# multiplefish/VPLines-SLAM

Measured on AMD Instinct MI355X. Metric: sliding-window BA solves/sec (10 KF, 200 pts + 80 lines, 5 iters), higher is better.
Workload: dtype f64

## Files before the change

vplines-slam_amd/csrc/ba_ctx.h:

```cpp
#pragma once
#include <functional>
#include <map>
#include <string>

#include "vplines_ba.h"
#include "ba_types.h"
#include "ba_stage.h"

struct vpl_ctx {
  int device = 0;
  hipStream_t stream = nullptr;
  DevBatch B;
  std::vector<DevAlloc> allocs;
  bool guards = false;
  std::string err;
  int maxW = 0, maxP = 0, maxPO = 0, maxL = 0, maxLO = 0;
  int nW = 0;
  vpl_ba_options opt;
  bool upload_open = false;
  std::vector<int> h_nP, h_nL;
  std::vector<std::vector<int>> h_lmap;
  std::vector<int> h_mg_m;
  std::vector<int> h_mg_n;
  std::vector<int> h_mg_nb;
  std::vector<int> h_passthrough;
  std::vector<vpl_prior> h_pass_priors;
  bool any_second_new = false;
  int maxPriorN = 0;
  bool prior_resident = false;
  int prior_resident_nW = 0;
  std::vector<int> layout_key;
  bool layout_valid = false;
  bool force_general = false;
  bool schur_mostly_wide = false;
  bool schur_never_wide = false;
  bool schur_wide_all = false;
  bool step_fused = true;
  size_t marg_smem = 0;
  int marg_nmax = 0;
  bool marg_small = false;
  int prior_rule = VPL_PRIOR_PIVOTED_CHOLESKY;
  hipGraphExec_t graph_exec = nullptr;
  bool use_graph = true;
  bool timing = false;
  std::map<std::string, std::pair<double, int>> ktimes;
  std::vector<std::pair<const char*, double>> ltimes;
  int* d_act = nullptr;
  std::vector<std::string> kname_store;
  bool leg_timing = false;
  hipEvent_t leg_ev[6] = {nullptr, nullptr, nullptr, nullptr, nullptr, nullptr};
  double odo_ms[3] = {0, 0, 0};
  std::function<int()> pending;
  Stage stage;
  size_t last_upload_bytes = 0;
  struct vpl_odo* odo = nullptr;
};

static void drop_graph(vpl_ctx* c) {
  if (c->graph_exec) { (void)hipGraphExecDestroy(c->graph_exec); c->graph_exec = nullptr; }
}

static int settle(vpl_ctx* c) {
  if (!c || !c->pending) return VPL_OK;
  std::function<int()> fin;
  fin.swap(c->pending);
  return fin();
}
static int finish_or_defer(vpl_ctx* c, bool async, std::function<int()> fin) {
  if (!async) return fin();
  c->pending = std::move(fin);
  return VPL_OK;
}

struct KTimer {
  vpl_ctx* c;
  const char* name;
  hipEvent_t a = nullptr, b = nullptr;
  KTimer(vpl_ctx* c_, const char* n) : c(c_), name(n) {
    if (c->timing) { (void)hipEventCreate(&a); (void)hipEventCreate(&b); (void)hipEventRecord(a, c->stream); }
  }
  ~KTimer() {
    if (c->timing) {
      (void)hipEventRecord(b, c->stream);
      (void)hipEventSynchronize(b);
      float ms = 0;
      (void)hipEventElapsedTime(&ms, a, b);
      auto& e = c->ktimes[name];
      e.first += ms;
      e.second += 1;
// ... 14 lines not shown
```

vplines-slam_amd/csrc/ba_lin.h:

```cpp
#pragma once
#include "ba_common.h"

namespace vpl {

typedef double v4d_lin __attribute__((ext_vector_type(4)));
constexpr int LIN_THREADS = 512;
constexpr int STG_LD = 17;
constexpr int LIN_STAGE = 8 * 32 * STG_LD;
constexpr int PRE_LDS = 62;
constexpr int LIN_HW = 720;
constexpr int PREP_NMAX = 112;
__host__ __device__ constexpr int lin_stage_doubles(int maxL) {
  const int ln = 8 * LIN_HW + 38 * maxL;
  const int pt = LIN_STAGE + 78 * 36 + NV;
  const int m = ln > pt ? ln : pt;
  return m > 4650 + 3570 ? m : 4650 + 3570;
}
constexpr int PREP_THREADS = 640;
inline size_t prep_smem(int max_prior_n) {
  const int ns = max_prior_n < PREP_NMAX ? max_prior_n : PREP_NMAX;
  return (size_t)((PREP_THREADS / 64) * 675 + ns * ns) * sizeof(double);
}
constexpr size_t PREP_SMEM = (size_t)((PREP_THREADS / 64) * 675 + PREP_NMAX * PREP_NMAX) * sizeof(double);

__device__ __forceinline__ void prep_body(const DevBatch& B, const int w, double* psm, int nstage) {
  const int tid = threadIdx.x;
  const int lane = tid & 63, wv = tid >> 6;
  const int NWV = blockDim.x >> 6;
  double* wsc = psm + wv * 675;
  double* Jl = psm + NWV * 675;
  const int n = B.pr_n[w];
  const bool fits = n > 0 && n <= nstage;
  if (fits) {
    const double* J0g = B.pr_J0 + (size_t)w * B.prS;
    for (int idx = tid; idx < n * n; idx += blockDim.x) Jl[idx] = J0g[idx];
  }
  for (int j = 1 + wv; j < NF; j += NWV) {
    DevPreint& P = B.pre[(size_t)w * NF + j];
    double* G = wsc;
    double* X = wsc + 225;
    double* Pm = wsc + 450;
    for (int k = lane; k < 225; k += 64) G[k] = P.cov[k];
    __builtin_amdgcn_wave_barrier();
    wave_chol16(G, 15, 15, X, lane);
    __builtin_amdgcn_wave_barrier();
    for (int e = lane; e < 225; e += 64) {
      const int a = e / 15, b2 = e % 15;
      double s2 = 0;
      for (int k = (a > b2 ? a : b2); k < 15; ++k) s2 += X[k * 15 + a] * X[k * 15 + b2];
      Pm[e] = s2;
    }
    __builtin_amdgcn_wave_barrier();
    wave_chol16(Pm, 15, 15, nullptr, lane);
    __builtin_amdgcn_wave_barrier();
    for (int e = lane; e < 225; e += 64) {
      const int i = e / 15, jj = e % 15;
      P.sqrt_info[e] = (jj >= i) ? Pm[jj * 15 + i] : 0.0;
    }
    __builtin_amdgcn_wave_barrier();
  }
  if (tid < NF + 1) {
    double* x = tid < NF ? B.pose + ((size_t)w * NF + tid) * 7 : B.ex + (size_t)w * 7;
    Q4 q = mat2q(qmat(qnormalized(qpose(x))));
    if (tid == 0) {
      M3 R0 = qmat(qnormalized(qpose(x)));
      V3 ypr = R2ypr(R0);
      double* g = B.gauge + (size_t)w * 4;
      g[0] = ypr.x; g[1] = x[0]; g[2] = x[1]; g[3] = x[2];
      const double* fr = B.fail_ref + (size_t)w * 13;
      if (fr[0] != 0.0) {
        M3 Rl;
        for (int k = 0; k < 9; ++k) Rl.m[k] = fr[4 + k];
        g[0] = R2ypr(Rl).x; g[1] = fr[1]; g[2] = fr[2]; g[3] = fr[3];
      }
    }
    x[3] = q.x; x[4] = q.y; x[5] = q.z; x[6] = q.w;
    double* xq = psm + 7 * tid;
    xq[0] = x[0]; xq[1] = x[1]; xq[2] = x[2]; xq[3] = q.x; xq[4] = q.y; xq[5] = q.z; xq[6] = q.w;
  }
  __syncthreads();
  const int nL = B.orth_in[w] ? 0 : B.nL[w];
  for (int l = tid; l < nL; l += blockDim.x) {
    const int s = B.ln_start[(size_t)w * B.maxL + l];
    const double* ps = psm + 7 * s;
    const double* ex = psm + 7 * NF;
    M3 Rs = qmat(qpose(ps)), ric = qmat(qpose(ex));
    V3 P{ps[0], ps[1], ps[2]}, tic{ex[0], ex[1], ex[2]};
    V3 twc = P + mul(Rs, tic);
    M3 Rwc = mul(Rs, ric);
    const double* pl = B.plk + ((size_t)w * B.maxL + l) * 6;
    Plk Lc{V3{pl[0], pl[1], pl[2]}, V3{pl[3], pl[4], pl[5]}};
    Plk Lw = plk_to_pose(Lc, Rwc, twc);
    plk_to_orth(Lw, B.orth + ((size_t)w * B.maxL + l) * 4);
  }
  for (int l = tid; l < B.nL[w]; l += blockDim.x) {
    const size_t li = (size_t)w * B.maxL + l;
    const Plk Lw = orth_to_plk(B.orth + li * 4);
    double* o = B.lw + li * 6;
    o[0] = Lw.n.x; o[1] = Lw.n.y; o[2] = Lw.n.z; o[3] = Lw.v.x; o[4] = Lw.v.y; o[5] = Lw.v.z;
  }
  if (n > 0) {
    const double* J0 = B.pr_J0 + (size_t)w * B.prS;
    double* H = B.pr_H + (size_t)w * B.prS;
    const double* Js = fits ? Jl : J0;
    if (fits) {
      const int NT = (n + 15) >> 4, NLT = NT * (NT + 1) / 2, KS = (n + 3) >> 2;
      const int m = lane & 15, kk = lane >> 4;
      for (int t = wv; t < NLT; t += NWV) {
        int ta, tb;
        tri_decode(t, ta, tb);
        const int ca = 16 * ta + m, cb = 16 * tb + m;
        v4d_lin acc = {0, 0, 0, 0};
        for (int ks = 0; ks < KS; ++ks) {
          const int k = 4 * ks + kk;
          const double av = (k < n && ca < n) ? Js[k * n + ca] : 0.0;
          const double bv = (k < n && cb < n) ? Js[k * n + cb] : 0.0;
          acc = __builtin_amdgcn_mfma_f64_16x16x4f64(av, bv, acc, 0, 0, 0);
        }
        const double vals[4] = {acc.x, acc.y, acc.z, acc.w};
#pragma unroll
        for (int v = 0; v < 4; ++v) {
          const int r = 16 * ta + kk + 4 * v, c2 = cb;
          if (r < n && c2 < n && (ta != tb || r >= c2)) {
            H[(size_t)r * n + c2] = vals[v];
            H[(size_t)c2 * n + r] = vals[v];
          }
        }
      }
    } else
    for (int idx = tid; idx < n * n; idx += blockDim.x) {
      int a = idx / n, b = idx % n;
      double s = 0;
      for (int k = 0; k < n; ++k) s += Js[(size_t)k * n + a] * Js[(size_t)k * n + b];
      H[idx] = s;
    }
    for (int c2 = tid; c2 < n; c2 += blockDim.x) {
      double s = 0;
      const double* r0g = B.pr_r0 + (size_t)w * MAXPN;
#pragma unroll 8
      for (int k = 0; k < n; ++k) s += Js[(size_t)k * n + c2] * r0g[k];
      B.pr_g0[(size_t)w * MAXPN + c2] = s;
    }
    if (tid < B.pr_nb[w]) {
      int kind = B.pr_kind[(size_t)w * MAXPB + tid], fr = B.pr_frame[(size_t)w * MAXPB + tid];
      int idx = B.pr_idx[(size_t)w * MAXPB + tid];
      int base = kind == 0 ? 15 * fr : kind == 1 ? 15 * fr + 6 : 165;
      int ls = kind == 1 ? 9 : 6;
      for (int k = 0; k < ls; ++k) B.pr_map[(size_t)w * MAXPN + idx + k] = base + k;
    }
  }
  if (tid == 0) {
    TrState t;
    t.radius = 1e4; t.mu = 1e-8; t.x_cost = 0; t.cand_cost = 0; t.model_cost_change = 0; t.x_norm = 0;
    t.step_norm = 0; t.dogleg_step_norm = 0; t.alpha = 0; t.a1 = t.a2 = t.a3 = 0; t.initial_cost = 0;
    t.iter = 0; t.status = 0; t.reuse = 0; t.step_valid = 0; t.fresh_lin = 0; t.num_successful = 0; t.num_invalid = 0;
    t.pad = 0;
    B.tr[w] = t;
  }
}
__global__ __launch_bounds__(PREP_THREADS) void k_prep(DevBatch B, int nstage) {
  extern __shared__ double psm[];
  prep_body(B, blockIdx.x, psm, nstage);
}

constexpr int HV_DOUBLES = 78 * 36;
constexpr int LIN_PART = 78 * 36 + 72 + 8;
__host__ __device__ __forceinline__ int hvi(int r, int c) {
  const int br = r / 6, bc = c / 6;
  return 36 * (br * (br + 1) / 2 + bc) + 6 * (r - 6 * br) + (c - 6 * bc);
}

inline void lin_asm_entry(int r, int c, int* out) {
  int hv = 0, im = 0;
  const int vr = cam2vis(r), vc = cam2vis(c);
  if (vr >= 0 && vc >= 0) hv = hvi(vr, vc) + 1;
  if (r < 165) {
    const int fr = r / 15, ar = r - 15 * fr, fc = c / 15, bc = c - 15 * fc;
    if (fc == fr) im = 120 * fr + ar * (ar + 1) / 2 + bc + 1;
    else if (fc == fr - 1) im = 11 * 120 + 225 * (fr - 1) + 15 * ar + bc + 1;
  }
  out[0] = hv | im << 16;
  out[1] = r | c << 8;
}

template <int MODE, int ROLE>
// ... 775 lines not shown
```

vplines-slam_amd/csrc/ba_upload.h:

```cpp
#pragma once
#include "ba_ctx.h"
#include "ba_odo.h"
#include "ba_pack.h"
#include "host_common.h"

static void to_dev_preint(const vpl_preintegration& p, DevPreint& d) {
  d.sum_dt = p.sum_dt;
  for (int k = 0; k < 3; ++k) { d.dp[k] = p.delta_p[k]; d.dv[k] = p.delta_v[k]; d.lba[k] = p.linearized_ba[k]; d.lbg[k] = p.linearized_bg[k]; }
  for (int k = 0; k < 4; ++k) d.dq[k] = p.delta_q[k];
  auto blk = [&](double* o, int r0, int c0) {
    for (int i = 0; i < 3; ++i)
      for (int j = 0; j < 3; ++j) o[3 * i + j] = p.jacobian[(r0 + i) * 15 + c0 + j];
  };
  blk(d.dp_dba, 0, 9); blk(d.dp_dbg, 0, 12); blk(d.dq_dbg, 3, 12); blk(d.dv_dba, 6, 9); blk(d.dv_dbg, 6, 12);
  std::memcpy(d.cov, p.covariance, sizeof(d.cov));
  std::memset(d.sqrt_info, 0, sizeof(d.sqrt_info));
}

struct UploadArena {
  Span<double> pose, sb, ex, invd, plk, pt_obs, ln_obs, fail_ref, orth, pr_x0, pr_r0;
  Span<int> nP, nL, pt_start, pt_nobs, pt_off, ln_start, ln_nobs, ln_off, ln_tri, pu_cnt, pu_cnt0, sk_tab, sk_wave, path, nLO, lo_ln,
      ll_tab, ll_np, ps_list, ps_cnt, orth_in, pr_n, pr_nb, pr_kind, pr_frame, pr_idx, mg_n, mg_nb, mg_kind, mg_frame, mg_idx, mg_cam, mg_m;
  Span<DevPreint> pre;
  std::vector<Span<double>> J0;
// ... 86 lines not shown
    for (size_t w = 0; w < W; ++w) S.put(B.pr_J0 + w * (size_t)B.prS, A.J0[w]);
  }
  S.put(B.mg_n, A.mg_n); S.put(B.mg_nb, A.mg_nb); S.put(B.mg_kind, A.mg_kind);
  S.put(B.mg_frame, A.mg_frame); S.put(B.mg_idx, A.mg_idx); S.put(B.mg_cam, A.mg_cam); S.put(B.mg_m, A.mg_m);
  S.put(B.path, A.path);
}
static size_t upload_bound(const DevBatch& B, size_t W, const vpl_window* win, bool same_layout, bool chained, const OdoSrc* odo) {
  Stage dry;
  dry.dry = true;
  UploadArena A;
  take_upload(dry, A, B, W, win, chained, odo);
  take_units(dry, A, W, B.maxPR);
  stage_upload(dry, A, B, W, same_layout, chained, odo);
  return dry.bound();
}

static int upload_check(vpl_ctx* c, int nW, const vpl_window* win, const vpl_ba_options* opt, bool chained) {
  if (!c || !win || !opt || nW < 1) return VPL_E_INVALID;
  if (nW > c->maxW) return fail(c, VPL_E_CAPACITY, "more windows than max_windows");
  if (opt->marginalization_flag != VPL_MARGIN_OLD && opt->marginalization_flag != VPL_MARGIN_SECOND_NEW &&
      opt->marginalization_flag != VPL_MARGIN_NONE)
    return fail(c, VPL_E_INVALID, "unknown marginalization_flag");
  HIPCHK(c, hipSetDevice(c->device));
  { const int rs = settle(c); if (rs) return rs; }
  if (chained && (!c->prior_resident || c->prior_resident_nW != nW))
    return fail(c, VPL_E_INVALID, "upload_chained: needs a previous solve of the same batch size with a marginalisation, and no upload since");
  return VPL_OK;
}

static int read_resident_priors(vpl_ctx* c, size_t W, std::vector<HostTab>& tab) {
  const DevBatch& B = c->B;
  int* const src[10] = {B.mg_n, B.mg_nb, B.mg_kind, B.mg_frame, B.mg_idx, B.pr_n, B.pr_nb, B.pr_kind, B.pr_frame, B.pr_idx};
  Span<int> t[10];
  auto plan = [&](Stage& S) {
    for (int k = 0; k < 10; ++k) {
      t[k] = S.take<int>(k % 5 < 2 ? W : W * MAXPB);
      S.from_device(t[k].p, src[k], t[k].n);
    }
  };
  HIPCHK(c, stage_plan(c->stage, plan));
  HIPCHK(c, stage_run(c->stage, c->stream, false));
  HIPCHK(c, hipStreamSynchronize(c->stream));
  tab.resize(W);
  for (size_t w = 0; w < W; ++w) {
    HostTab& T = tab[w];
    T.keep = c->h_passthrough[w] >= 0;
    const Span<int>* s = t + (T.keep ? 5 : 0);
// ... 258 lines not shown
  DevBuf dkeep;
  HIPCHK(c, dkeep.alloc(nW * 4));
  HIPCHK(c, hipMemcpyAsync(dkeep.p, keep.data(), nW * 4, hipMemcpyHostToDevice, c->stream));
  if (B.prS != prev_prS && std::any_of(keep.begin(), keep.end(), [](int k) { return k != 0; })) {
    DevBuf tmp;
    HIPCHK(c, tmp.alloc(nW * (size_t)MAXPN * MAXPN * 8));
    hipLaunchKernelGGL(k_prior_restride, dim3(nW), dim3(256), 0, c->stream, B, (const int*)dkeep.p, prev_prS, tmp.d(), 0);
    hipLaunchKernelGGL(k_prior_restride, dim3(nW), dim3(256), 0, c->stream, B, (const int*)dkeep.p, prev_prS, tmp.d(), 1);
    HIPCHK(c, hipGetLastError());
    HIPCHK(c, hipStreamSynchronize(c->stream));
  }
  hipLaunchKernelGGL(k_prior_handoff, dim3(nW), dim3(256), 0, c->stream, B, (const int*)dkeep.p);
  HIPCHK(c, hipGetLastError());
  HIPCHK(c, hipStreamSynchronize(c->stream));
  return VPL_OK;
}

static int upload_body(vpl_ctx* c, int nW, const vpl_window* win, const vpl_ba_options* opt, bool all_lines, bool chained,
                       const OdoSrc* odo) {
  int rc = upload_check(c, nW, win, opt, chained);
  if (rc) return rc;
  const int prev_prS = c->B.prS;
  c->prior_resident = false;
  if (c->leg_timing) HIPCHK(c, hipEventRecord(c->leg_ev[0], c->stream));
  drop_graph(c);
  c->upload_open = true;
  c->opt = *opt;
  c->nW = nW;
  DevBatch& B = c->B;
  B.nW = nW;
  B.opt.num_iterations = opt->num_iterations;
  B.opt.estimate_extrinsic = opt->estimate_extrinsic;
  B.opt.marginalization_flag = opt->marginalization_flag;
  B.opt.remove_line_outliers = opt->remove_line_outliers;
  B.opt.sqrt_info_point = opt->focal_length / 1.5;
  B.opt.sqrt_info_line = opt->line_factor;
  B.opt.sqrt_info_vp = opt->vp_factor;
  B.opt.g_norm = opt->g_norm;
  B.opt.huber_delta = opt->huber_delta;
  const size_t W = nW;
  std::vector<HostTab> ctab;
  if (chained && (rc = read_resident_priors(c, W, ctab))) return rc;
  const bool dev_prior = chained || odo;
  if (odo) {
    ctab.assign(W, HostTab());
    for (size_t w = 0; w < W; ++w)
// ... 39 lines not shown
  if (SG.overflow) return fail(c, VPL_E_CAPACITY, "internal: staging arena bound too small");
  stage_upload(SG, A, B, W, same_layout, dev_prior, odo);
  if (chained && (rc = hand_over_priors(c, ctab, prev_prS))) return rc;
  HIPCHK(c, stage_run(c->stage, c->stream, true, &c->last_upload_bytes));
  if (odo) {
    hipLaunchKernelGGL(k_odo_gather, dim3(nW), dim3(ODO_THREADS), 0, c->stream, B, odo->store, (const int*)odo->d_psrc, (const int*)odo->d_lsrc);
    if (odo->tab) hipLaunchKernelGGL(k_odo_prior_load, dim3(nW), dim3(ODO_THREADS), 0, c->stream, B, odo->prior, (const int*)odo->d_has);
    HIPCHK(c, hipGetLastError());
  }
  if (c->leg_timing) HIPCHK(c, hipEventRecord(c->leg_ev[1], c->stream));
  HIPCHK(c, hipStreamSynchronize(c->stream));
  c->layout_valid = true;
  return VPL_OK;
}
static int upload_impl(vpl_ctx* c, int nW, const vpl_window* win, const vpl_ba_options* opt, bool all_lines, bool chained = false,
                       const OdoSrc* odo = nullptr) {
  const int rc = upload_body(c, nW, win, opt, all_lines, chained, odo);
  if (c) {
    if (rc != VPL_OK && c->upload_open) { c->nW = 0; c->prior_resident = false; }
    c->upload_open = false;
  }
  return rc;
}

static int restore_states(vpl_ctx* c, bool plk) {
  const DevBatch& B = c->B;
  const size_t W = c->nW;
  HIPCHK(c, hipMemcpyAsync(B.pose, B.pose_0, W * 77 * 8, hipMemcpyDeviceToDevice, c->stream));
  HIPCHK(c, hipMemcpyAsync(B.sb, B.sb_0, W * 99 * 8, hipMemcpyDeviceToDevice, c->stream));
  HIPCHK(c, hipMemcpyAsync(B.ex, B.ex_0, W * 7 * 8, hipMemcpyDeviceToDevice, c->stream));
  HIPCHK(c, hipMemcpyAsync(B.invd, B.invd_0, W * B.maxP * 8, hipMemcpyDeviceToDevice, c->stream));
  if (plk) HIPCHK(c, hipMemcpyAsync(B.plk, B.plk_0, W * B.maxL * 6 * 8, hipMemcpyDeviceToDevice, c->stream));
  return VPL_OK;
}
```

vplines-slam_amd/csrc/vplines_ba.hip:

```cpp
#include <hip/hip_runtime.h>

#include <algorithm>
#include <chrono>
#include <memory>
#include <cstdlib>
#include <cstring>
#include <string>
#include <vector>

#include "vplines_ba.h"
#include "ba_types.h"
#include "ba_lin.h"
#include "ba_pack.h"
#include "ba_solve.h"
#include "ba_step.h"
#include "ba_marg.h"
#include "ba_prior_eig.h"
#include "ba_lineopt.h"
#include "ba_factors.h"
#include "ba_odo.h"
#include "odo_tracks.h"
#include "host_common.h"

using namespace vpl;
// ... 138 lines not shown
      }
    if ((int)nz.size() != NZ_N || hipMemcpy(B.nz_tab, nz.data(), nz.size() * sizeof(int), hipMemcpyHostToDevice) != hipSuccess) return VPL_E_HIP;
  }
  static size_t lin_max = 0, solve_max = 0, schur_max = 0, back_max = 0, step_max = 0;
  lin_max = std::max(lin_max, lin_smem(c->maxP, c->maxL));
  solve_max = std::max(solve_max, solve_smem(c->maxP, c->maxL));
  schur_max = std::max(schur_max, schur_smem(c->maxP, c->maxL));
  back_max = std::max(back_max, back_smem(c->maxP, c->maxL));
  step_max = std::max(step_max, step_smem(c->maxP, c->maxL));
  if (schur_max > 159 * 1024 || back_max > 159 * 1024) return VPL_E_CAPACITY;
  const std::pair<const void*, size_t> lds[] = {
      {(const void*)k_lin2, lin_max}, {(const void*)k_lin<1>, lin_max}, {(const void*)k_lin<2>, lin_max},
      {(const void*)k_solve, solve_max}, {(const void*)k_schur<3>, schur_max}, {(const void*)k_schur<5>, schur_max},
      {(const void*)k_schur_mixed, schur_max}, {(const void*)k_chol, CHOL_SMEM}, {(const void*)k_back, back_max},
      {(const void*)k_step<3, false>, step_max}, {(const void*)k_step<3, true>, step_max}, {(const void*)k_step<5, false>, step_max},
      {(const void*)k_prep, PREP_SMEM}, {(const void*)k_marg<MARG_THREADS>, 159 * 1024}, {(const void*)k_marg<256>, MARG_LDS_SMALL},
      {(const void*)k_prior_eigen, prior_eig_layout(MAXKEEP).bytes}, {(const void*)k_init_align, init_lds_bytes(INIT_NMAX)}};
  for (const auto& k : lds)
    if (hipFuncSetAttribute(k.first, hipFuncAttributeMaxDynamicSharedMemorySize, (int)k.second) != hipSuccess) return VPL_E_HIP;
  vpl_ba_default_options(&c->opt);
  if (const char* gv = std::getenv("VPL_BA_GRAPH")) c->use_graph = std::atoi(gv) != 0;
  if (const char* gv = std::getenv("VPL_BA_GENERAL")) c->force_general = std::atoi(gv) != 0;
  if (const char* gv = std::getenv("VPL_BA_STEP_FUSED")) c->step_fused = std::atoi(gv) != 0;
  if (const char* gv = std::getenv("VPL_BA_SCHUR_WIDE")) { c->schur_wide_all = std::atoi(gv) > 0; c->schur_never_wide = std::atoi(gv) < 0; }
  return VPL_OK;
}

int vpl_ctx_create(vpl_ctx** out, int device, int max_windows, int max_points, int max_point_obs, int max_lines,
                   int max_line_obs) {
  if (!out || max_windows < 1 || max_points < 0 || max_lines < 0) return VPL_E_INVALID;
  int ndev = 0;
  if (hipGetDeviceCount(&ndev) != hipSuccess || ndev == 0 || device >= ndev) return VPL_E_NODEVICE;
  if (hipSetDevice(device) != hipSuccess) return VPL_E_NODEVICE;
  vpl_ctx* c = new vpl_ctx();
  const int rc = ctx_init(c, device, max_windows, max_points, max_point_obs, max_lines, max_line_obs);
  if (rc != VPL_OK) {
    free_arrays(c);
    delete c;
    return rc;
  }
  *out = c;
  return VPL_OK;
}

void vpl_ctx_destroy(vpl_ctx* c) {
  if (!c) return;
  (void)hipSetDevice(c->device);
  (void)hipDeviceSynchronize();
  drop_graph(c);
  free_arrays(c);
  c->stage.release();
  for (hipEvent_t& e : c->leg_ev) if (e) (void)hipEventDestroy(e);
  delete c;
}

int vpl_ctx_set_stream(vpl_ctx* c, void* s) {
  if (!c) return VPL_E_INVALID;
  const int rs = settle(c);
  if (rs) return rs;
  if (c->stream != (hipStream_t)s) {
    HIPCHK(c, hipSetDevice(c->device));
    (void)hipStreamSynchronize(c->stream);
    (void)hipGetLastError();
  }
  drop_graph(c);
  c->stream = (hipStream_t)s;
  return VPL_OK;
}
int vpl_ba_set_prior_rule(vpl_ctx* c, int rule) {
  if (!c || (rule != VPL_PRIOR_PIVOTED_CHOLESKY && rule != VPL_PRIOR_EIGEN)) return VPL_E_INVALID;
  const int rs = settle(c);
  if (rs) return rs;
  drop_graph(c);
  c->prior_rule = rule;
  return VPL_OK;
}
const char* vpl_last_error(const vpl_ctx* c) { return c ? c->err.c_str() : "null context"; }

int vpl_ctx_enable_leg_timing(vpl_ctx* c, int enable) {
  if (!c) return VPL_E_INVALID;
  HIPCHK(c, hipSetDevice(c->device));
  if (enable)
    for (hipEvent_t& e : c->leg_ev) if (!e) HIPCHK(c, hipEventCreate(&e));
  c->leg_timing = enable != 0;
  return VPL_OK;
}
int vpl_ctx_leg_times(vpl_ctx* c, double* ms3) {
  if (!c || !ms3 || !c->leg_timing) return VPL_E_INVALID;
  HIPCHK(c, hipSetDevice(c->device));
  HIPCHK(c, hipStreamSynchronize(c->stream));
// ... 107 lines not shown
  HIPCHK(c, hipMemcpyAsync(dJ.p, pr->J0, (size_t)n * n * 8, hipMemcpyHostToDevice, c->stream));
  HIPCHK(c, hipMemcpyAsync(dr0.p, pr->r0, n * 8, hipMemcpyHostToDevice, c->stream));
  HIPCHK(c, hipMemcpyAsync(dp.p, params, psz * 8, hipMemcpyHostToDevice, c->stream));
  hipLaunchKernelGGL(k_eval_prior, dim3(1), dim3(256), 0, c->stream, n, nb, (const int*)dk.p, (const int*)di.p, dx0.d(),
                     dJ.d(), dr0.d(), dp.d(), dr.d(), jac ? dj.d() : nullptr);
  HIPCHK(c, hipGetLastError());
  HIPCHK(c, hipMemcpyAsync(residuals, dr.p, n * 8, hipMemcpyDeviceToHost, c->stream));
  if (jac) HIPCHK(c, hipMemcpyAsync(jac, dj.p, (size_t)n * psz * 8, hipMemcpyDeviceToHost, c->stream));
  HIPCHK(c, hipStreamSynchronize(c->stream));
  return VPL_OK;
}
int vpl_pose_plus(vpl_ctx* c, int n, const double* x, const double* delta, double* out) {
  return eval_generic(c, n, x, 7, delta, 6, 7, 0, out, nullptr, [&](double* p, double* k, double* r, double*) {
    hipLaunchKernelGGL(k_eval_pose_plus, dim3((n + 63) / 64), dim3(64), 0, c->stream, n, p, k, r);
  });
}
int vpl_line_orth_plus(vpl_ctx* c, int n, const double* x, const double* delta, double* out) {
  return eval_generic(c, n, x, 4, delta, 4, 4, 0, out, nullptr, [&](double* p, double* k, double* r, double*) {
    hipLaunchKernelGGL(k_eval_orth_plus, dim3((n + 63) / 64), dim3(64), 0, c->stream, n, p, k, r);
  });
}

int vpl_ba_reset_state(vpl_ctx* c) {
  if (c) { const int rs = settle(c); if (rs) return rs; }
  if (!c || c->nW < 1) return VPL_E_INVALID;
  return restore_states(c, true);
}

int vpl_ba_upload(vpl_ctx* c, int nW, const vpl_window* win, const vpl_ba_options* opt) {
  return upload_impl(c, nW, win, opt, false);
}
int vpl_ba_upload_chained(vpl_ctx* c, int nW, const vpl_window* win, const vpl_ba_options* opt) {
  return upload_impl(c, nW, win, opt, false, true);
}

static void launch_prep(vpl_ctx* c, const DevBatch& B, int nw, hipStream_t s) {
  KTimer t(c, "k_prep");
  hipLaunchKernelGGL(k_prep, dim3(nw), dim3(PREP_THREADS), prep_smem(c->maxPriorN), s, B, std::min(c->maxPriorN, PREP_NMAX));
}
static void launch_marg(vpl_ctx* c, DevBatch& B, int nw, hipStream_t s) {
  const bool old = c->opt.marginalization_flag == VPL_MARGIN_OLD;
  if (!old && !c->any_second_new) return;
  const dim3 grid(nw);
  { KTimer t(c, "k_lin_marg");
    if (old) hipLaunchKernelGGL(k_lin<1>, grid, dim3(LIN_THREADS), lin_smem(c->maxP, c->maxL), s, B);
    else hipLaunchKernelGGL(k_lin<2>, grid, dim3(LIN_THREADS), lin_smem(c->maxP, c->maxL), s, B); }
  ++B.launch;
  { KTimer t(c, "k_marg");
    if (c->marg_small) hipLaunchKernelGGL(k_marg<256>, grid, dim3(256), c->marg_smem, s, B);
    else hipLaunchKernelGGL(k_marg<MARG_THREADS>, grid, dim3(MARG_THREADS), c->marg_smem, s, B); }
  if (c->prior_rule == VPL_PRIOR_EIGEN) {
    KTimer t(c, "k_prior_eigen");
    hipLaunchKernelGGL(k_prior_eigen, grid, dim3(PRIOR_EIG_THREADS), prior_eig_layout(c->marg_nmax).bytes, s, B, c->marg_nmax);
  }
}
static void launch_triangulate(vpl_ctx* c, int nW, bool points, bool lines, double init_depth) {
  const DevBatch& B = c->B;
  hipStream_t s = c->stream;
  if (points) { KTimer t(c, "k_triangulate_points"); hipLaunchKernelGGL(k_triangulate_points, dim3(nW), dim3(128), 0, s, B, init_depth); }
  if (lines) { KTimer t(c, "k_triangulate"); hipLaunchKernelGGL(k_triangulate, dim3(nW), dim3(128), 0, s, B); }
}
// ... 190 lines not shown
    for (size_t w = 0; w < W; ++w) {
      vpl_window& v = win[w];
      if (reports) std::memset(&reports[w], 0, sizeof(reports[w]));
      if (c->h_lmap[w].size() < 4) {
        if (v.line_removed) std::fill(v.line_removed, v.line_removed + v.n_lines, 0);
        continue;
      }
      const int nrem = scatter_solved_lines(c, w, v, &(*plk)[w * maxL * 6], &(*removed)[w * maxL]);
      if (reports) {
        fill_report(reports[w], (*tr)[w]);
        reports[w].n_lines_removed = nrem;
      }
    }
    return VPL_OK;
  });
}
int vpl_ba_only_line_opt(vpl_ctx* c, int nW, vpl_window* win, const vpl_ba_options* opt, vpl_solve_report* reports) {
  return only_line_opt_impl(c, nW, win, opt, reports, false);
}
int vpl_ba_only_line_opt_async(vpl_ctx* c, int nW, vpl_window* win, const vpl_ba_options* opt, vpl_solve_report* reports) {
  return only_line_opt_impl(c, nW, win, opt, reports, true);
}

static void launch_solve(vpl_ctx* c, int w0, int nw, hipStream_t s) {
  DevBatch B = c->B;
  B.ord_it = 0;
  B.act = c->timing ? c->d_act : nullptr;
  B.launch = 0;
  B.step_fused = c->step_fused && !c->timing;
  if (c->timing) { c->ltimes.clear(); (void)hipMemsetAsync(c->d_act, 0, sizeof(int) * ACT_SLOTS * 4, s); }
  const dim3 grid(nw);
  launch_prep(c, B, nw, s);
  ++B.launch;
  { KTimer t(c, "k_lin"); hipLaunchKernelGGL(k_lin2, dim3(16 * ((nw + 7) / 8)), dim3(LIN_THREADS), lin_smem(c->maxP, c->maxL), s, B); }
  ++B.launch;
  for (int it = 0; it < c->opt.num_iterations; ++it) {
    B.ord_it = it;
    const bool wide = c->schur_wide_all || (c->schur_mostly_wide && !c->schur_never_wide);
    if (B.step_fused) {
      if (B.WS + 2 <= 48) hipLaunchKernelGGL((k_step<3, false>), grid, dim3(SCHUR_THREADS), step_smem(B.maxP, B.maxL, 3), s, B);
      else if (wide) hipLaunchKernelGGL((k_step<5, false>), grid, dim3(SCHUR_THREADS), step_smem(B.maxP, B.maxL, 5), s, B);
      else hipLaunchKernelGGL((k_step<3, true>), grid, dim3(SCHUR_THREADS), step_smem(B.maxP, B.maxL, 3), s, B);
      ++B.launch;
      hipLaunchKernelGGL(k_solve, grid, dim3(SOLVE_THREADS), solve_smem(B.maxP, B.maxL), s, B);
      ++B.launch;
    } else {
      { KTimer t(c, "k_schur");
        if (B.WS + 2 <= 48) hipLaunchKernelGGL(k_schur<3>, grid, dim3(SCHUR_THREADS), schur_smem(B.maxP, B.maxL, 3), s, B);
        else if (wide) hipLaunchKernelGGL(k_schur<5>, grid, dim3(SCHUR_THREADS), schur_smem(B.maxP, B.maxL, 5), s, B);
        else hipLaunchKernelGGL(k_schur_mixed, grid, dim3(SCHUR_THREADS), schur_smem(B.maxP, B.maxL, 3), s, B); }
      ++B.launch;
      { KTimer t(c, "k_chol"); hipLaunchKernelGGL(k_chol, grid, dim3(CHOL_THREADS), CHOL_SMEM, s, B); }
      ++B.launch;
      { KTimer t(c, "k_solve"); hipLaunchKernelGGL(k_solve, grid, dim3(SOLVE_THREADS), solve_smem(B.maxP, B.maxL), s, B); }
      ++B.launch;
      { KTimer t(c, "k_back"); hipLaunchKernelGGL(k_back, grid, dim3(BACK_THREADS), back_smem(B.maxP, B.maxL), s, B); }
      ++B.launch;
    }
    { KTimer t(c, "k_cost"); hipLaunchKernelGGL(k_cost, grid, dim3(COST_THREADS), 0, s, B); }
    ++B.launch;
    if (it + 1 < c->opt.num_iterations) {
      B.ord_it = it + 1;
      KTimer t(c, "k_lin");
      hipLaunchKernelGGL(k_lin2, dim3(16 * ((nw + 7) / 8)), dim3(LIN_THREADS), lin_smem(c->maxP, c->maxL), s, B);
    }
    if (it + 1 < c->opt.num_iterations) ++B.launch;
  }
  B.ord_it = 0;
  { KTimer t(c, "k_gauge"); hipLaunchKernelGGL(k_gauge, grid, dim3(128), 0, s, B); }
  ++B.launch;
  launch_marg(c, B, nw, s);
}

int vpl_ba_solve(vpl_ctx* c) {
  if (c) { const int rs = settle(c); if (rs) return rs; }
  if (!c || c->nW < 1) return VPL_E_INVALID;
  HIPCHK(c, hipSetDevice(c->device));
  if (c->opt.marginalization_flag != VPL_MARGIN_NONE) { c->prior_resident = true; c->prior_resident_nW = c->nW; }
  if (c->leg_timing) {
    HIPCHK(c, hipEventRecord(c->leg_ev[2], c->stream));
    launch_solve(c, 0, c->nW, c->stream);
    HIPCHK(c, hipGetLastError());
    HIPCHK(c, hipEventRecord(c->leg_ev[3], c->stream));
    return VPL_OK;
  }
  if (c->use_graph && !c->timing && c->stream != nullptr) {
    if (!c->graph_exec) {
      hipGraph_t graph = nullptr;
      HIPCHK(c, hipStreamBeginCapture(c->stream, hipStreamCaptureModeThreadLocal));
      launch_solve(c, 0, c->nW, c->stream);
      HIPCHK(c, hipStreamEndCapture(c->stream, &graph));
      hipError_t e = hipGraphInstantiate(&c->graph_exec, graph, nullptr, nullptr, 0);
      (void)hipGraphDestroy(graph);
      if (e != hipSuccess) { c->graph_exec = nullptr; return fail(c, VPL_E_HIP, std::string("hipGraphInstantiate: ") + hipGetErrorString(e)); }
    }
    HIPCHK(c, hipGraphLaunch(c->graph_exec, c->stream));
    return VPL_OK;
  }
  launch_solve(c, 0, c->nW, c->stream);
  HIPCHK(c, hipGetLastError());
  return VPL_OK;
}

struct PriorFetch {
  Span<int> mg_n, mg_nb, mg_kind, mg_frame, mg_idx, mg_m;
  Span<double> mg_x0, mg_r0;
  std::vector<Span<double>> J0;
};
static void prior_fetch_plan(vpl_ctx* c, int nW, PriorFetch& F, Stage& S) {
  const DevBatch& B = c->B;
  const size_t W = nW;
  F.mg_m = S.take<int>(W); F.mg_n = S.take<int>(W); F.mg_nb = S.take<int>(W);
  F.mg_kind = S.take<int>(W * MAXPB); F.mg_frame = S.take<int>(W * MAXPB); F.mg_idx = S.take<int>(W * MAXPB);
  F.mg_x0 = S.take<double>(W * MAXPB * 9); F.mg_r0 = S.take<double>(W * MAXKEEP);
  S.from_device(F.mg_m.p, B.mg_m, W); S.from_device(F.mg_n.p, B.mg_n, W); S.from_device(F.mg_nb.p, B.mg_nb, W);
  S.from_device(F.mg_kind.p, B.mg_kind, W * MAXPB); S.from_device(F.mg_frame.p, B.mg_frame, W * MAXPB);
  S.from_device(F.mg_idx.p, B.mg_idx, W * MAXPB);
  S.from_device(F.mg_x0.p, B.mg_x0, W * MAXPB * 9); S.from_device(F.mg_r0.p, B.mg_r0, W * MAXKEEP);
  F.J0.resize(W);
  for (size_t w = 0; w < W; ++w) {
    const int n = w < c->h_mg_n.size() ? std::min(std::max(c->h_mg_n[w], 0), (int)MAXKEEP) : (int)MAXKEEP;
    F.J0[w] = S.take<double>((size_t)n * n);
// ... 141 lines not shown
}
int vpl_ba_marginalize(vpl_ctx* c, int nW, const vpl_window* win, const vpl_ba_options* opt, int marginalization_flag,
                       vpl_prior* priors, int* m_out, int* n_out) {
  return marginalize_impl(c, nW, win, opt, marginalization_flag, priors, m_out, n_out, false);
}
int vpl_ba_marginalize_async(vpl_ctx* c, int nW, const vpl_window* win, const vpl_ba_options* opt, int marginalization_flag,
                             vpl_prior* priors, int* m_out, int* n_out) {
  return marginalize_impl(c, nW, win, opt, marginalization_flag, priors, m_out, n_out, true);
}

int vpl_ba_solve_windows(vpl_ctx* c, int nW, vpl_window* win, const vpl_ba_options* opt, vpl_prior* priors,
                         vpl_solve_report* reports) {
  int rc = vpl_ba_upload(c, nW, win, opt);
  if (rc) return rc;
  rc = vpl_ba_solve(c);
  if (rc) return rc;
  rc = vpl_ctx_synchronize(c);
  if (rc) return rc;
  return vpl_ba_download(c, nW, win, priors, reports);
}

static int reuse_line_opt_batch(vpl_ctx* c) {
  HIPCHK(c, hipMemsetAsync(c->B.ln_removed, 0, (size_t)c->nW * c->B.maxL * 4, c->stream));
  return restore_states(c, false);
}

int vpl_ba_solve_odometry(vpl_ctx* c, int nW, vpl_window* win, const vpl_ba_options* opt, double init_depth,
                          vpl_prior* priors, vpl_solve_report* line_reports, vpl_solve_report* reports) {
  if (!c || !win || !opt || nW < 1) return VPL_E_INVALID;
  bool any_lines = false;
  for (int w = 0; w < nW; ++w)
    if (win[w].n_lines > 0) {
      any_lines = true;
      if (!win[w].line_triangulated || !win[w].line_removed)
        return fail(c, VPL_E_INVALID, "solve_odometry: line_triangulated and line_removed are required for windows with lines");
    }
  using oclk = std::chrono::steady_clock;
  const auto t0 = oclk::now();
  int rc = triangulate_impl(c, nW, win, true, any_lines, init_depth, false);
  if (rc) return rc;
  const auto t1 = oclk::now();
  c->odo_ms[0] = std::chrono::duration<double, std::milli>(t1 - t0).count();
  c->odo_ms[1] = 0.0;
  bool batch_resident = false;
  if (any_lines) {
    bool orth_given = false;
    for (int w = 0; w < nW; ++w) orth_given = orth_given || win[w].line_orth != nullptr;
// ... 152 lines not shown
```

Baseline: 264,700.

## Fold state-restore memcpys into prep kernel via deferred restore state machine

Instead of issuing four or five device-to-device memcpys on reset_state and reuse, the restore request is recorded and folded into the k_prep kernel, which reads from the *_0 snapshots directly. A separate graph executable is cached per restore mode. Prep also hoists the prior r0 vector into shared memory and prefetches line/covariance data before the syncthreads. This removes several small copy launches per solve, at the cost of more state-machine complexity and extra graph instantiations.

```diff
diff --git a/vplines-slam_amd/csrc/ba_ctx.h b/vplines-slam_amd/csrc/ba_ctx.h
--- a/vplines-slam_amd/csrc/ba_ctx.h
+++ b/vplines-slam_amd/csrc/ba_ctx.h
@@ -6,6 +6,7 @@
 #include "vplines_ba.h"
 #include "ba_types.h"
 #include "ba_stage.h"
+#include "ba_restore.h"
 
 struct vpl_ctx {
   int device = 0;
@@ -40,8 +41,10 @@
   int marg_nmax = 0;
   bool marg_small = false;
   int prior_rule = VPL_PRIOR_PIVOTED_CHOLESKY;
-  hipGraphExec_t graph_exec = nullptr;
+  hipGraphExec_t graph_exec[3] = {nullptr, nullptr, nullptr};
   bool use_graph = true;
+  int restore_pending = RESTORE_NONE;
+  bool restore_fold = true;
   bool timing = false;
   std::map<std::string, std::pair<double, int>> ktimes;
   std::vector<std::pair<const char*, double>> ltimes;
@@ -57,14 +60,40 @@
 };
 
 static void drop_graph(vpl_ctx* c) {
-  if (c->graph_exec) { (void)hipGraphExecDestroy(c->graph_exec); c->graph_exec = nullptr; }
+  for (hipGraphExec_t& g : c->graph_exec)
+    if (g) { (void)hipGraphExecDestroy(g); g = nullptr; }
 }
 
-static int settle(vpl_ctx* c) {
+static int restore_states(vpl_ctx* c, int mode) {
+  if (mode == RESTORE_NONE || c->nW < 1) return VPL_OK;
+  const DevBatch& B = c->B;
+  const size_t W = c->nW;
+  HIPCHK(c, hipSetDevice(c->device));
+  HIPCHK(c, hipMemcpyAsync(B.pose, B.pose_0, W * 77 * 8, hipMemcpyDeviceToDevice, c->stream));
+  HIPCHK(c, hipMemcpyAsync(B.sb, B.sb_0, W * 99 * 8, hipMemcpyDeviceToDevice, c->stream));
+  HIPCHK(c, hipMemcpyAsync(B.ex, B.ex_0, W * 7 * 8, hipMemcpyDeviceToDevice, c->stream));
+  HIPCHK(c, hipMemcpyAsync(B.invd, B.invd_0, W * B.maxP * 8, hipMemcpyDeviceToDevice, c->stream));
+  if (mode == RESTORE_LINES) HIPCHK(c, hipMemcpyAsync(B.plk, B.plk_0, W * B.maxL * 6 * 8, hipMemcpyDeviceToDevice, c->stream));
+  return VPL_OK;
+}
+static int restore_event(vpl_ctx* c, RestoreEvent ev, int* prep = nullptr) {
+  const RestoreStep s = restore_step(c->restore_pending, ev, c->restore_fold);
+  c->restore_pending = s.pending;
+  if (prep) *prep = s.prep;
+  return restore_states(c, s.flush);
+}
+
+static int settle_call(vpl_ctx* c) {
   if (!c || !c->pending) return VPL_OK;
   std::function<int()> fin;
   fin.swap(c->pending);
   return fin();
+}
+static int settle(vpl_ctx* c) {
+  if (!c) return VPL_OK;
+  const int rs = settle_call(c);
+  if (rs) return rs;
+  return restore_event(c, RESTORE_EV_OBSERVE);
 }
 static int finish_or_defer(vpl_ctx* c, bool async, std::function<int()> fin) {
   if (!async) return fin();
diff --git a/vplines-slam_amd/csrc/ba_lin.h b/vplines-slam_amd/csrc/ba_lin.h
--- a/vplines-slam_amd/csrc/ba_lin.h
+++ b/vplines-slam_amd/csrc/ba_lin.h
@@ -19,28 +19,94 @@
 constexpr int PREP_THREADS = 640;
 inline size_t prep_smem(int max_prior_n) {
   const int ns = max_prior_n < PREP_NMAX ? max_prior_n : PREP_NMAX;
-  return (size_t)((PREP_THREADS / 64) * 675 + ns * ns) * sizeof(double);
-}
-constexpr size_t PREP_SMEM = (size_t)((PREP_THREADS / 64) * 675 + PREP_NMAX * PREP_NMAX) * sizeof(double);
-
-__device__ __forceinline__ void prep_body(const DevBatch& B, const int w, double* psm, int nstage) {
+  return (size_t)((PREP_THREADS / 64) * 675 + ns * ns + ns + 84) * sizeof(double);
+}
+constexpr size_t PREP_SMEM = (size_t)((PREP_THREADS / 64) * 675 + PREP_NMAX * PREP_NMAX + PREP_NMAX + 84) * sizeof(double);
+
+__device__ __forceinline__ void prep_body(const DevBatch& B, const int w, double* psm, int nstage, const int restore) {
   const int tid = threadIdx.x;
   const int lane = tid & 63, wv = tid >> 6;
   const int NWV = blockDim.x >> 6;
   double* wsc = psm + wv * 675;
   double* Jl = psm + NWV * 675;
+  double* r0s = Jl + nstage * nstage;
+  double* xq = r0s + nstage;
+  const int nrs = restore ? 99 + B.maxP + (restore > 1 ? 6 * B.maxL : 0) : 0;
+  auto rs_src = [&](int i) -> const double* {
+    return i < 99 ? B.sb_0 + (size_t)w * 99 + i
+                  : i < 99 + B.maxP ? B.invd_0 + (size_t)w * B.maxP + (i - 99) : B.plk_0 + (size_t)w * B.maxL * 6 + (i - 99 - B.maxP);
+  };
+  auto rs_dst = [&](int i) -> double* {
+    return i < 99 ? B.sb + (size_t)w * 99 + i
+                  : i < 99 + B.maxP ? B.invd + (size_t)w * B.maxP + (i - 99) : B.plk + (size_t)w * B.maxL * 6 + (i - 99 - B.maxP);
+  };
+  const int rs1 = tid + (int)blockDim.x;
+  double rv0 = 0.0, rv1 = 0.0;
+  if (tid < nrs) rv0 = *rs_src(tid);
+  if (rs1 < nrs) rv1 = *rs_src(rs1);
   const int n = B.pr_n[w];
   const bool fits = n > 0 && n <= nstage;
   if (fits) {
     const double* J0g = B.pr_J0 + (size_t)w * B.prS;
     for (int idx = tid; idx < n * n; idx += blockDim.x) Jl[idx] = J0g[idx];
-  }
+    const double* r0g = B.pr_r0 + (size_t)w * MAXPN;
+    for (int idx = tid; idx < n; idx += blockDim.x) r0s[idx] = r0g[idx];
+  }
+  const int nLw = B.nL[w];
+  const bool orth_in = B.orth_in[w] != 0;
+  const double* plk_in = (restore > 1 ? B.plk_0 : B.plk) + (size_t)w * B.maxL * 6;
+  int s1 = 0;
+  double pl1[6] = {0, 0, 0, 0, 0, 0};
+  if (!orth_in && tid < nLw) {
+    s1 = B.ln_start[(size_t)w * B.maxL + tid];
+#pragma unroll
+    for (int q = 0; q < 6; ++q) pl1[q] = plk_in[tid * 6 + q];
+  }
+  double cv[4] = {0, 0, 0, 0};
+  if (1 + wv < NF) {
+    const DevPreint& P1 = B.pre[(size_t)w * NF + 1 + wv];
+#pragma unroll
+    for (int i = 0; i < 4; ++i)
+      if (lane + 64 * i < 225) cv[i] = P1.cov[lane + 64 * i];
+  }
+  if (tid < nrs) *rs_dst(tid) = rv0;
+  if (rs1 < nrs) *rs_dst(rs1) = rv1;
+  for (int i = rs1 + (int)blockDim.x; i < nrs; i += blockDim.x) *rs_dst(i) = *rs_src(i);
+  if (tid < NF + 1) {
+    double* x = tid < NF ? B.pose + ((size_t)w * NF + tid) * 7 : B.ex + (size_t)w * 7;
+    const double* xin = !restore ? x : tid < NF ? B.pose_0 + ((size_t)w * NF + tid) * 7 : B.ex_0 + (size_t)w * 7;
+    const double x0 = xin[0], x1 = xin[1], x2 = xin[2];
+    Q4 q = mat2q(qmat(qnormalized(qpose(xin))));
+    if (tid == 0) {
+      M3 R0 = qmat(qnormalized(qpose(xin)));
+      V3 ypr = R2ypr(R0);
+      double* g = B.gauge + (size_t)w * 4;
+      g[0] = ypr.x; g[1] = x0; g[2] = x1; g[3] = x2;
+      const double* fr = B.fail_ref + (size_t)w * 13;
+      if (fr[0] != 0.0) {
+        M3 Rl;
+        for (int k = 0; k < 9; ++k) Rl.m[k] = fr[4 + k];
+        g[0] = R2ypr(Rl).x; g[1] = fr[1]; g[2] = fr[2]; g[3] = fr[3];
+      }
+    }
+    if (restore) { x[0] = x0; x[1] = x1; x[2] = x2; }
+    x[3] = q.x; x[4] = q.y; x[5] = q.z; x[6] = q.w;
+    double* xo = xq + 7 * tid;
+    xo[0] = x0; xo[1] = x1; xo[2] = x2; xo[3] = q.x; xo[4] = q.y; xo[5] = q.z; xo[6] = q.w;
+  }
+  __syncthreads();
   for (int j = 1 + wv; j < NF; j += NWV) {
     DevPreint& P = B.pre[(size_t)w * NF + j];
     double* G = wsc;
     double* X = wsc + 225;
     double* Pm = wsc + 450;
-    for (int k = lane; k < 225; k += 64) G[k] = P.cov[k];
+    if (j == 1 + wv) {
+#pragma unroll
+      for (int i = 0; i < 4; ++i)
+        if (lane + 64 * i < 225) G[lane + 64 * i] = cv[i];
+    } else {
+      for (int k = lane; k < 225; k += 64) G[k] = P.cov[k];
+    }
     __builtin_amdgcn_wave_barrier();
     wave_chol16(G, 15, 15, X, lane);
     __builtin_amdgcn_wave_barrier();
@@ -59,43 +125,31 @@
     }
     __builtin_amdgcn_wave_barrier();
   }
-  if (tid < NF + 1) {
-    double* x = tid < NF ? B.pose + ((size_t)w * NF + tid) * 7 : B.ex + (size_t)w * 7;
-    Q4 q = mat2q(qmat(qnormalized(qpose(x))));
-    if (tid == 0) {
-      M3 R0 = qmat(qnormalized(qpose(x)));
-      V3 ypr = R2ypr(R0);
-      double* g = B.gauge + (size_t)w * 4;
-      g[0] = ypr.x; g[1] = x[0]; g[2] = x[1]; g[3] = x[2];
-      const double* fr = B.fail_ref + (size_t)w * 13;
-      if (fr[0] != 0.0) {
-        M3 Rl;
-        for (int k = 0; k < 9; ++k) Rl.m[k] = fr[4 + k];
-        g[0] = R2ypr(Rl).x; g[1] = fr[1]; g[2] = fr[2]; g[3] = fr[3];
-      }
-    }
-    x[3] = q.x; x[4] = q.y; x[5] = q.z; x[6] = q.w;
-    double* xq = psm + 7 * tid;
-    xq[0] = x[0]; xq[1] = x[1]; xq[2] = x[2]; xq[3] = q.x; xq[4] = q.y; xq[5] = q.z; xq[6] = q.w;
-  }
-  __syncthreads();
-  const int nL = B.orth_in[w] ? 0 : B.nL[w];
-  for (int l = tid; l < nL; l += blockDim.x) {
-    const int s = B.ln_start[(size_t)w * B.maxL + l];
-    const double* ps = psm + 7 * s;
-    const double* ex = psm + 7 * NF;
-    M3 Rs = qmat(qpose(ps)), ric = qmat(qpose(ex));
-    V3 P{ps[0], ps[1], ps[2]}, tic{ex[0], ex[1], ex[2]};
-    V3 twc = P + mul(Rs, tic);
-    M3 Rwc = mul(Rs, ric);
-    const double* pl = B.plk + ((size_t)w * B.maxL + l) * 6;
-    Plk Lc{V3{pl[0], pl[1], pl[2]}, V3{pl[3], pl[4], pl[5]}};
-    Plk Lw = plk_to_pose(Lc, Rwc, twc);
-    plk_to_orth(Lw, B.orth + ((size_t)w * B.maxL + l) * 4);
-  }
-  for (int l = tid; l < B.nL[w]; l += blockDim.x) {
+  for (int l = tid; l < nLw; l += blockDim.x) {
     const size_t li = (size_t)w * B.maxL + l;
-    const Plk Lw = orth_to_plk(B.orth + li * 4);
+    double o4[4];
+    if (!orth_in) {
+      const bool first = l == tid;
+      const int s = first ? s1 : B.ln_start[li];
+      const double* ps = xq + 7 * s;
+      const double* ex = xq + 7 * NF;
+      M3 Rs = qmat(qpose(ps)), ric = qmat(qpose(ex));
+      V3 P{ps[0], ps[1], ps[2]}, tic{ex[0], ex[1], ex[2]};
+      V3 twc = P + mul(Rs, tic);
+      M3 Rwc = mul(Rs, ric);
+      double pl[6];
+#pragma unroll
+      for (int q = 0; q < 6; ++q) pl[q] = first ? pl1[q] : plk_in[(size_t)l * 6 + q];
+      Plk Lc{V3{pl[0], pl[1], pl[2]}, V3{pl[3], pl[4], pl[5]}};
+      Plk Lw = plk_to_pose(Lc, Rwc, twc);
+      plk_to_orth(Lw, o4);
+      double* og = B.orth + li * 4;
+      og[0] = o4[0]; og[1] = o4[1]; og[2] = o4[2]; og[3] = o4[3];
+    } else {
+      const double* og = B.orth + li * 4;
+      o4[0] = og[0]; o4[1] = og[1]; o4[2] = og[2]; o4[3] = og[3];
+    }
+    const Plk Lw = orth_to_plk(o4);
     double* o = B.lw + li * 6;
     o[0] = Lw.n.x; o[1] = Lw.n.y; o[2] = Lw.n.z; o[3] = Lw.v.x; o[4] = Lw.v.y; o[5] = Lw.v.z;
   }
@@ -136,9 +190,14 @@
     }
     for (int c2 = tid; c2 < n; c2 += blockDim.x) {
       double s = 0;
-      const double* r0g = B.pr_r0 + (size_t)w * MAXPN;
+      if (fits) {
 #pragma unroll 8
-      for (int k = 0; k < n; ++k) s += Js[(size_t)k * n + c2] * r0g[k];
+        for (int k = 0; k < n; ++k) s += Jl[k * n + c2] * r0s[k];
+      } else {
+        const double* r0g = B.pr_r0 + (size_t)w * MAXPN;
+#pragma unroll 8
+        for (int k = 0; k < n; ++k) s += J0[(size_t)k * n + c2] * r0g[k];
+      }
       B.pr_g0[(size_t)w * MAXPN + c2] = s;
     }
     if (tid < B.pr_nb[w]) {
@@ -158,9 +217,9 @@
     B.tr[w] = t;
   }
 }
-__global__ __launch_bounds__(PREP_THREADS) void k_prep(DevBatch B, int nstage) {
+__global__ __launch_bounds__(PREP_THREADS) void k_prep(DevBatch B, int nstage, int restore) {
   extern __shared__ double psm[];
-  prep_body(B, blockIdx.x, psm, nstage);
+  prep_body(B, blockIdx.x, psm, nstage, restore);
 }
 
 constexpr int HV_DOUBLES = 78 * 36;
diff --git a/vplines-slam_amd/csrc/ba_restore.h b/vplines-slam_amd/csrc/ba_restore.h
--- /dev/null
+++ b/vplines-slam_amd/csrc/ba_restore.h
@@ -0,0 +1,44 @@
+#pragma once
+
+enum RestoreMode { RESTORE_NONE = 0, RESTORE_STATES = 1, RESTORE_LINES = 2 };
+
+enum RestoreEvent {
+  RESTORE_EV_RESET,
+  RESTORE_EV_REUSE,
+  RESTORE_EV_SOLVE,
+  RESTORE_EV_UPLOAD,
+  RESTORE_EV_OBSERVE,
+  RESTORE_EV_DESTROY
+};
+
+struct RestoreStep {
+  int flush;
+  int prep;
+  int pending;
+};
+
+inline RestoreStep restore_step(int pending, RestoreEvent ev, bool fold) {
+  RestoreStep s = {RESTORE_NONE, RESTORE_NONE, pending};
+  switch (ev) {
+    case RESTORE_EV_RESET:
+    case RESTORE_EV_REUSE: {
+      const int want = ev == RESTORE_EV_RESET ? RESTORE_LINES : RESTORE_STATES;
+      if (!fold) { s.flush = want; s.pending = RESTORE_NONE; }
+      else s.pending = pending > want ? pending : want;
+      break;
+    }
+    case RESTORE_EV_SOLVE:
+      s.prep = pending;
+      s.pending = RESTORE_NONE;
+      break;
+    case RESTORE_EV_UPLOAD:
+    case RESTORE_EV_DESTROY:
+      s.pending = RESTORE_NONE;
+      break;
+    case RESTORE_EV_OBSERVE:
+      s.flush = pending;
+      s.pending = RESTORE_NONE;
+      break;
+  }
+  return s;
+}
diff --git a/vplines-slam_amd/csrc/ba_upload.h b/vplines-slam_amd/csrc/ba_upload.h
--- a/vplines-slam_amd/csrc/ba_upload.h
+++ b/vplines-slam_amd/csrc/ba_upload.h
@@ -132,7 +132,7 @@
       opt->marginalization_flag != VPL_MARGIN_NONE)
     return fail(c, VPL_E_INVALID, "unknown marginalization_flag");
   HIPCHK(c, hipSetDevice(c->device));
-  { const int rs = settle(c); if (rs) return rs; }
+  { const int rs = settle_call(c); if (rs) return rs; }
   if (chained && (!c->prior_resident || c->prior_resident_nW != nW))
     return fail(c, VPL_E_INVALID, "upload_chained: needs a previous solve of the same batch size with a marginalisation, and no upload since");
   return VPL_OK;
@@ -437,6 +437,7 @@
   if (rc) return rc;
   const int prev_prS = c->B.prS;
   c->prior_resident = false;
+  (void)restore_event(c, RESTORE_EV_UPLOAD);
   if (c->leg_timing) HIPCHK(c, hipEventRecord(c->leg_ev[0], c->stream));
   drop_graph(c);
   c->upload_open = true;
@@ -522,14 +523,3 @@
   }
   return rc;
 }
-
-static int restore_states(vpl_ctx* c, bool plk) {
-  const DevBatch& B = c->B;
-  const size_t W = c->nW;
-  HIPCHK(c, hipMemcpyAsync(B.pose, B.pose_0, W * 77 * 8, hipMemcpyDeviceToDevice, c->stream));
-  HIPCHK(c, hipMemcpyAsync(B.sb, B.sb_0, W * 99 * 8, hipMemcpyDeviceToDevice, c->stream));
-  HIPCHK(c, hipMemcpyAsync(B.ex, B.ex_0, W * 7 * 8, hipMemcpyDeviceToDevice, c->stream));
-  HIPCHK(c, hipMemcpyAsync(B.invd, B.invd_0, W * B.maxP * 8, hipMemcpyDeviceToDevice, c->stream));
-  if (plk) HIPCHK(c, hipMemcpyAsync(B.plk, B.plk_0, W * B.maxL * 6 * 8, hipMemcpyDeviceToDevice, c->stream));
-  return VPL_OK;
-}
diff --git a/vplines-slam_amd/csrc/vplines_ba.hip b/vplines-slam_amd/csrc/vplines_ba.hip
--- a/vplines-slam_amd/csrc/vplines_ba.hip
+++ b/vplines-slam_amd/csrc/vplines_ba.hip
@@ -184,6 +184,7 @@
   if (const char* gv = std::getenv("VPL_BA_GRAPH")) c->use_graph = std::atoi(gv) != 0;
   if (const char* gv = std::getenv("VPL_BA_GENERAL")) c->force_general = std::atoi(gv) != 0;
   if (const char* gv = std::getenv("VPL_BA_STEP_FUSED")) c->step_fused = std::atoi(gv) != 0;
+  if (const char* gv = std::getenv("VPL_BA_RESET_FOLD")) c->restore_fold = std::atoi(gv) != 0;
   if (const char* gv = std::getenv("VPL_BA_SCHUR_WIDE")) { c->schur_wide_all = std::atoi(gv) > 0; c->schur_never_wide = std::atoi(gv) < 0; }
   return VPL_OK;
 }
@@ -209,6 +210,7 @@
   if (!c) return;
   (void)hipSetDevice(c->device);
   (void)hipDeviceSynchronize();
+  (void)restore_event(c, RESTORE_EV_DESTROY);
   drop_graph(c);
   free_arrays(c);
   c->stage.release();
@@ -218,7 +220,7 @@
 
 int vpl_ctx_set_stream(vpl_ctx* c, void* s) {
   if (!c) return VPL_E_INVALID;
-  const int rs = settle(c);
+  const int rs = settle_call(c);
   if (rs) return rs;
   if (c->stream != (hipStream_t)s) {
     HIPCHK(c, hipSetDevice(c->device));
@@ -227,7 +229,7 @@
   }
   drop_graph(c);
   c->stream = (hipStream_t)s;
-  return VPL_OK;
+  return restore_event(c, RESTORE_EV_OBSERVE);
 }
 int vpl_ba_set_prior_rule(vpl_ctx* c, int rule) {
   if (!c || (rule != VPL_PRIOR_PIVOTED_CHOLESKY && rule != VPL_PRIOR_EIGEN)) return VPL_E_INVALID;
@@ -381,9 +383,9 @@
 }
 
 int vpl_ba_reset_state(vpl_ctx* c) {
-  if (c) { const int rs = settle(c); if (rs) return rs; }
+  if (c) { const int rs = settle_call(c); if (rs) return rs; }
   if (!c || c->nW < 1) return VPL_E_INVALID;
-  return restore_states(c, true);
+  return restore_event(c, RESTORE_EV_RESET);
 }
 
 int vpl_ba_upload(vpl_ctx* c, int nW, const vpl_window* win, const vpl_ba_options* opt) {
@@ -393,9 +395,9 @@
   return upload_impl(c, nW, win, opt, false, true);
 }
 
-static void launch_prep(vpl_ctx* c, const DevBatch& B, int nw, hipStream_t s) {
+static void launch_prep(vpl_ctx* c, const DevBatch& B, int nw, hipStream_t s, int restore = RESTORE_NONE) {
   KTimer t(c, "k_prep");
-  hipLaunchKernelGGL(k_prep, dim3(nw), dim3(PREP_THREADS), prep_smem(c->maxPriorN), s, B, std::min(c->maxPriorN, PREP_NMAX));
+  hipLaunchKernelGGL(k_prep, dim3(nw), dim3(PREP_THREADS), prep_smem(c->maxPriorN), s, B, std::min(c->maxPriorN, PREP_NMAX), restore);
 }
 static void launch_marg(vpl_ctx* c, DevBatch& B, int nw, hipStream_t s) {
   const bool old = c->opt.marginalization_flag == VPL_MARGIN_OLD;
@@ -632,7 +634,7 @@
   return only_line_opt_impl(c, nW, win, opt, reports, true);
 }
 
-static void launch_solve(vpl_ctx* c, int w0, int nw, hipStream_t s) {
+static void launch_solve(vpl_ctx* c, int w0, int nw, hipStream_t s, int restore) {
   DevBatch B = c->B;
   B.ord_it = 0;
   B.act = c->timing ? c->d_act : nullptr;
@@ -640,7 +642,7 @@
   B.step_fused = c->step_fused && !c->timing;
   if (c->timing) { c->ltimes.clear(); (void)hipMemsetAsync(c->d_act, 0, sizeof(int) * ACT_SLOTS * 4, s); }
   const dim3 grid(nw);
-  launch_prep(c, B, nw, s);
+  launch_prep(c, B, nw, s, restore);
   ++B.launch;
   { KTimer t(c, "k_lin"); hipLaunchKernelGGL(k_lin2, dim3(16 * ((nw + 7) / 8)), dim3(LIN_THREADS), lin_smem(c->maxP, c->maxL), s, B); }
   ++B.launch;
@@ -683,31 +685,34 @@
 }
 
 int vpl_ba_solve(vpl_ctx* c) {
-  if (c) { const int rs = settle(c); if (rs) return rs; }
+  if (c) { const int rs = settle_call(c); if (rs) return rs; }
   if (!c || c->nW < 1) return VPL_E_INVALID;
   HIPCHK(c, hipSetDevice(c->device));
+  int restore = RESTORE_NONE;
+  { const int rr = restore_event(c, RESTORE_EV_SOLVE, &restore); if (rr) return rr; }
   if (c->opt.marginalization_flag != VPL_MARGIN_NONE) { c->prior_resident = true; c->prior_resident_nW = c->nW; }
   if (c->leg_timing) {
     HIPCHK(c, hipEventRecord(c->leg_ev[2], c->stream));
-    launch_solve(c, 0, c->nW, c->stream);
+    launch_solve(c, 0, c->nW, c->stream, restore);
     HIPCHK(c, hipGetLastError());
     HIPCHK(c, hipEventRecord(c->leg_ev[3], c->stream));
     return VPL_OK;
   }
   if (c->use_graph && !c->timing && c->stream != nullptr) {
-    if (!c->graph_exec) {
+    hipGraphExec_t& exec = c->graph_exec[restore];
+    if (!exec) {
       hipGraph_t graph = nullptr;
       HIPCHK(c, hipStreamBeginCapture(c->stream, hipStreamCaptureModeThreadLocal));
-      launch_solve(c, 0, c->nW, c->stream);
+      launch_solve(c, 0, c->nW, c->stream, restore);
       HIPCHK(c, hipStreamEndCapture(c->stream, &graph));
-      hipError_t e = hipGraphInstantiate(&c->graph_exec, graph, nullptr, nullptr, 0);
+      hipError_t e = hipGraphInstantiate(&exec, graph, nullptr, nullptr, 0);
       (void)hipGraphDestroy(graph);
-      if (e != hipSuccess) { c->graph_exec = nullptr; return fail(c, VPL_E_HIP, std::string("hipGraphInstantiate: ") + hipGetErrorString(e)); }
-    }
-    HIPCHK(c, hipGraphLaunch(c->graph_exec, c->stream));
+      if (e != hipSuccess) { exec = nullptr; return fail(c, VPL_E_HIP, std::string("hipGraphInstantiate: ") + hipGetErrorString(e)); }
+    }
+    HIPCHK(c, hipGraphLaunch(exec, c->stream));
     return VPL_OK;
   }
-  launch_solve(c, 0, c->nW, c->stream);
+  launch_solve(c, 0, c->nW, c->stream, restore);
   HIPCHK(c, hipGetLastError());
   return VPL_OK;
 }
@@ -895,7 +900,7 @@
 
 static int reuse_line_opt_batch(vpl_ctx* c) {
   HIPCHK(c, hipMemsetAsync(c->B.ln_removed, 0, (size_t)c->nW * c->B.maxL * 4, c->stream));
-  return restore_states(c, false);
+  return restore_event(c, RESTORE_EV_REUSE);
 }
 
 int vpl_ba_solve_odometry(vpl_ctx* c, int nW, vpl_window* win, const vpl_ba_options* opt, double init_depth,
```

Result: faster. 268,300, median of 6 (+1.4%).
